# d8ahazard/AudioLab

Hardware: AMD Instinct MI355X
Metric: stems*realtime-factor (44.1kHz stereo) (higher is better)
Workload: dtype bf16; 1 GPU; MDX-Net UVR 4-stem (4x TFC-TDF U-Net L=11 g=48 dim_f=3072 dim_t=256 n_fft=6144), 300 s 44.1 kHz stereo in total, margin chunker, windows/launch=52; stems=4

## Files before the change

audiolab_amd/csrc/tdfnet.hip:

```cpp
#include "mma.h"
#include <alsep_gfx950_asm.h>

#include <map>
#include <type_traits>

namespace {

constexpr int kThreads = 256;

template <typename T> struct Vec16;
template <> struct Vec16<float> { static constexpr int N = 4; };
template <> struct Vec16<bf16_t> { static constexpr int N = 8; };
__device__ __forceinline__ void store_vec(float* p, const float* y) { *reinterpret_cast<float4*>(p) = make_float4(y[0], y[1], y[2], y[3]); }
__device__ __forceinline__ void store_vec(bf16_t* p, const float* y) {
    bf16x8 q;
#pragma unroll
    for (int e = 0; e < 8; ++e) q[e] = (bf16_t)y[e];
    *reinterpret_cast<bf16x8*>(p) = q;
}
__device__ __forceinline__ void load_vec(const float* p, float* x) {
    const float4 q = *reinterpret_cast<const float4*>(p);
    x[0] = q.x; x[1] = q.y; x[2] = q.z; x[3] = q.w;
}
__device__ __forceinline__ void load_vec(const bf16_t* p, float* x) {
// ... 1652 lines not shown
#pragma unroll
            for (int mi = 0; mi < 3; ++mi) acc[u][ni][mi] = f32x4{0.f, 0.f, 0.f, 0.f};

    const int trow = l15 >> 2, tcol = (l15 & 3) * 4;
    const bf16_t* xlane = ring + (4 * lq + trow) * Tc::UC + tcol;
    auto mma_unit = [&](int u, const bf16x8 (&xf)[3], int par, int ks) {
#pragma unroll
        for (int ni = 0; ni < 3; ++ni)
#pragma unroll
            for (int mi = 0; mi < 3; ++mi) mma_step(acc[u][ni][mi], xf[ni], wf[(ALSEP_TDF_ABL & 1) ? 0 : par][ks][mi]);
    };
#define ALSEP_TDFW_STEP(it_, S_, P_)                                                              \
    do {                                                                                          \
        wait_vmcnt<Tc::GLDS>();                 \
        if ((it_) + 1 >= ntile) wait_vmcnt<0>();          \
        barrier_nodrain();                  \
        if ((it_) + 1 < ntile && !(ALSEP_TDF_ABL & 1)) issue_w((it_) + 1, 1 - (P_));              \
        if ((it_) + 2 < ntile && !(ALSEP_TDF_ABL & 4)) issue_x((it_) + 2, ((S_) + 2) % 3);        \
        const bf16_t* xs_ = xlane + (size_t)(S_) * Tc::STAGE_ELEMS;                               \
        bf16x8 xa[3], xb[3];                                                                      \
        tdfw_read_x<0, 0>(xa, xs_);                                                               \
        tdfw_read_x<0, 1>(xb, xs_);                                                               \
        lds_read_tr16_wait_n<6>();  mma_unit(0, xa, P_, 0);                                       \
        tdfw_read_x<0, 2>(xa, xs_);                                                               \
        lds_read_tr16_wait_n<6>();  mma_unit(1, xb, P_, 0);                                       \
        tdfw_read_x<0, 3>(xb, xs_);                                                               \
        lds_read_tr16_wait_n<6>();  mma_unit(2, xa, P_, 0);                                       \
        tdfw_read_x<1, 0>(xa, xs_);                                                               \
        lds_read_tr16_wait_n<6>();  mma_unit(3, xb, P_, 0);                                       \
        tdfw_read_x<1, 1>(xb, xs_);                                                               \
        lds_read_tr16_wait_n<6>();  mma_unit(0, xa, P_, 1);                                       \
        tdfw_read_x<1, 2>(xa, xs_);                                                               \
        lds_read_tr16_wait_n<6>();  mma_unit(1, xb, P_, 1);                                       \
        tdfw_read_x<1, 3>(xb, xs_);                                                               \
        lds_read_tr16_wait_n<6>();  mma_unit(2, xa, P_, 1);                                       \
        lds_read_tr16_wait_n<0>();  mma_unit(3, xb, P_, 1);                                       \
    } while (0)
    issue_x(0, 0);
    issue_w(0, 0);
    if (1 < ntile) issue_x(1, 1);
    for (int it = 0; it < ntile; it += 6) {
        ALSEP_TDFW_STEP(it, 0, 0);
        if (it + 1 < ntile) ALSEP_TDFW_STEP(it + 1, 1, 1);
        if (it + 2 < ntile) ALSEP_TDFW_STEP(it + 2, 2, 0);
        if (it + 3 < ntile) ALSEP_TDFW_STEP(it + 3, 0, 1);
        if (it + 4 < ntile) ALSEP_TDFW_STEP(it + 4, 1, 0);
        if (it + 5 < ntile) ALSEP_TDFW_STEP(it + 5, 2, 1);
    }
#undef ALSEP_TDFW_STEP
    wait_vmcnt<0>();
#pragma unroll
    for (int i = 0; i < 12; ++i) keep_vgprs_live(wf[i / 6][(i / 3) % 2][i % 3]);
    barrier_nodrain();

    float* stg = reinterpret_cast<float*>(alsep_smem) + (size_t)wave * (Tc::TR * Tc::SS);
    bf16_t* frow = reinterpret_cast<bf16_t*>(alsep_smem + Tc::stage_bytes) + (size_t)wave * (Tc::TR * Tc::FS);
    float* fwl = reinterpret_cast<float*>(alsep_smem + Tc::stage_bytes + Tc::final_bytes) + wave * Tc::FWN;
    float fw[3], fbs[4];
    if (FINAL) {
#pragma unroll
        for (int j = 0; j < 3; ++j) fw[j] = FW[j * 64 + lane];
#pragma unroll
        for (int r = 0; r < 4; ++r) fbs[r] = FB[r];
    }
    float bvv[3];
#pragma unroll
    for (int mi = 0; mi < 3; ++mi) bvv[mi] = bias ? bias[rowblk * Tc::TR + mi * 16 + l15] : 0.f;
    auto unit_base = [&](int u) {
        const int64_t U = u0 + u;
        return ((U / upc) * M + rowblk * Tc::TR) * (int64_t)C + (int)(U % upc) * Tc::UC;
    };
    unsigned loff[5];
#pragma unroll
    for (int it = 0; it < 5; ++it) {
        const int gidx = it * 64 + lane;
        loff[it] = (unsigned)(((gidx / 6) * C + (gidx % 6) * 8) * (int)sizeof(bf16_t));
    }
    constexpr int PF = RESIDUAL ? RPF : 0;
    bf16x8 rr[Tc::UN][5];
    auto load_res = [&](int u) {
        const ALSEP_GLOBAL char* rb = opaque_uniform_gptr(reinterpret_cast<const char*>(R + unit_base(u)));
#pragma unroll
        for (int it = 0; it < 5; ++it)
            if (it * 64 + lane < Tc::TR * 6) rr[u][it] = *reinterpret_cast<const ALSEP_GLOBAL bf16x8*>(rb + loff[it]);
    };
    if (RESIDUAL && !(ALSEP_TDF_ABL & 2)) {
#pragma unroll
        for (int u = 0; u < PF && u < Tc::UN; ++u) {
            load_res(u);
            if (FINAL && u == 0) {
#pragma unroll
                for (int j = 0; j < 3; ++j) fwl[j * 64 + lane] = fw[j];
            }
        }
    }
#pragma unroll
    for (int u = 0; u < Tc::UN; ++u) {
        const int cb = (int)((u0 + u) % upc) * Tc::UC;
        if (RESIDUAL && u + PF < Tc::UN && !(ALSEP_TDF_ABL & 2)) load_res(u + PF);
        ALSEP_GLOBAL char* yb = const_cast<ALSEP_GLOBAL char*>(opaque_uniform_gptr(reinterpret_cast<const char*>(Y + unit_base(u))));
#pragma unroll
        for (int ni = 0; ni < 3; ++ni) {
            const f32x4 sc = *reinterpret_cast<const f32x4*>(scale + cb + ni * 16 + 4 * lq);
            const f32x4 sh = *reinterpret_cast<const f32x4*>(shift + cb + ni * 16 + 4 * lq);
#pragma unroll
            for (int mi = 0; mi < 3; ++mi) {
                f32x4 v;
#pragma unroll
                for (int r = 0; r < 4; ++r) v[r] = fmaxf(fmaf(acc[u][ni][mi][r] + bvv[mi], sc[r], sh[r]), 0.f);
                *reinterpret_cast<f32x4*>(stg + (mi * 16 + l15) * Tc::SS + ni * 16 + 4 * lq) = v;
            }
        }
        __builtin_amdgcn_wave_barrier();
#pragma unroll
        for (int it = 0; it < 5; ++it) {
            const int gidx = it * 64 + lane;
            const int fr = gidx / 6, cg = gidx % 6;
            if (gidx < Tc::TR * 6) {
                const f32x4 lo = *reinterpret_cast<const f32x4*>(stg + fr * Tc::SS + cg * 8);
                const f32x4 hi = *reinterpret_cast<const f32x4*>(stg + fr * Tc::SS + cg * 8 + 4);
                float y[8] = {lo[0], lo[1], lo[2], lo[3], hi[0], hi[1], hi[2], hi[3]};
                if (RESIDUAL) {
#pragma unroll
                    for (int e = 0; e < 8; ++e) y[e] += (float)rr[u][it][e];
                }
                bf16x8 q;
#pragma unroll
                for (int e = 0; e < 8; ++e) q[e] = (bf16_t)y[e];
                if (FINAL) *reinterpret_cast<bf16x8*>(frow + fr * Tc::FS + cg * 8) = q;
                else stream_store(reinterpret_cast<ALSEP_GLOBAL bf16x8*>(yb + loff[it]), q);
            }
        }
        __builtin_amdgcn_wave_barrier();
        if (FINAL) {
            const int frl = lane < Tc::TR ? lane : Tc::TR - 1;
            float y[4] = {fbs[0], fbs[1], fbs[2], fbs[3]};
#pragma unroll 2
            for (int ci = 0; ci < Tc::UC; ci += 8) {
                const bf16x8 xv = *reinterpret_cast<const bf16x8*>(frow + frl * Tc::FS + ci);
#pragma unroll
                for (int r = 0; r < 4; ++r) {
                    const f32x4 w0 = *reinterpret_cast<const f32x4*>(fwl + r * Tc::UC + ci);
                    const f32x4 w1 = *reinterpret_cast<const f32x4*>(fwl + r * Tc::UC + ci + 4);
#pragma unroll
                    for (int e = 0; e < 4; ++e) y[r] = fmaf(w0[e], (float)xv[e], y[r]);
#pragma unroll
                    for (int e = 0; e < 4; ++e) y[r] = fmaf(w1[e], (float)xv[4 + e], y[r]);
                }
            }
#pragma unroll
            for (int r = 0; r < 4; ++r) y[r] *= falpha;
            if (lane < Tc::TR) store4(FOUT + (((u0 + u) * M + rowblk * Tc::TR + lane) << 2), y);
            __builtin_amdgcn_wave_barrier();
        }
    }
}

struct Ds48 { static constexpr int C = 48, M = 96, MS = M + 4, K = 192, MT = 6, KS = 6; };
__device__ __forceinline__ vec16 lds_read16_align8(const bf16_t* p) {
    struct alignas(8) half16 { uint32_t w[2]; };
    const half16 a = *reinterpret_cast<const half16*>(p), b = *reinterpret_cast<const half16*>(p + 4);
    vec16 v;
    v.w[0] = a.w[0]; v.w[1] = a.w[1]; v.w[2] = b.w[0]; v.w[3] = b.w[1];
    return v;
}

__global__ void __launch_bounds__(kThreads, 1)
ds48_stream_kernel(const bf16_t* __restrict__ X, bf16_t* __restrict__ Y, const bf16_t* __restrict__ Wf,
                   const float* __restrict__ scale, const float* __restrict__ shift, int64_t npix, int Tp, int Fp) {
    typedef Ds48 D;
    const int tid = threadIdx.x, lane = tid & 63, wave = tid >> 6;
    const int l15 = lane & 15, lq = lane >> 4;
    bf16_t* stg = reinterpret_cast<bf16_t*>(alsep_smem) + (size_t)wave * 64 * D::MS;
    bf16x8 wf[D::MT][D::KS];
#pragma unroll
    for (int mt = 0; mt < D::MT; ++mt)
#pragma unroll
        for (int ks = 0; ks < D::KS; ++ks)
            wf[mt][ks] = *reinterpret_cast<const bf16x8*>(Wf + ((size_t)(mt * D::KS + ks) * 64 + lane) * 8);
    float sc[D::MT][4], sh[D::MT][4];
#pragma unroll
    for (int mt = 0; mt < D::MT; ++mt)
#pragma unroll
        for (int r = 0; r < 4; ++r) { sc[mt][r] = scale[mt * 16 + 4 * lq + r]; sh[mt][r] = shift[mt * 16 + 4 * lq + r]; }
    const int64_t ntile = npix / 64;
    for (int64_t tile = (int64_t)blockIdx.x * 4 + wave; tile < ntile; tile += (int64_t)gridDim.x * 4) {
        const int64_t p0 = tile * 64;
        const int64_t fp0 = p0 % Fp, tp = (p0 / Fp) % Tp, bb = p0 / ((int64_t)Fp * Tp);
        const bf16_t* xrow = X + ((bb * 2 * Tp + 2 * tp) * (2 * (int64_t)Fp) + 2 * fp0) * D::C;
        f32x4 acc[D::MT][4];
#pragma unroll
        for (int mt = 0; mt < D::MT; ++mt)
#pragma unroll
            for (int ni = 0; ni < 4; ++ni) acc[mt][ni] = f32x4{0.f, 0.f, 0.f, 0.f};
#pragma unroll
        for (int ks = 0; ks < D::KS; ++ks) {
            const int k = ks * 32 + lq * 8;
            const int dy = k / (2 * D::C), rem = k % (2 * D::C);
            bf16x8 xf[4];
#pragma unroll
            for (int ni = 0; ni < 4; ++ni)
                xf[ni] = *reinterpret_cast<const bf16x8*>(xrow + (int64_t)dy * (2 * (int64_t)Fp * D::C) + (int64_t)(ni * 16 + l15) * (2 * D::C) + rem);
#pragma unroll
            for (int mt = 0; mt < D::MT; ++mt)
#pragma unroll
                for (int ni = 0; ni < 4; ++ni) mma_step(acc[mt][ni], wf[mt][ks], xf[ni]);
        }
#pragma unroll
        for (int mt = 0; mt < D::MT; ++mt)
#pragma unroll
            for (int ni = 0; ni < 4; ++ni) {
                float y[4];
#pragma unroll
                for (int r = 0; r < 4; ++r) y[r] = fmaxf(fmaf(acc[mt][ni][r], sc[mt][r], sh[mt][r]), 0.f);
                store4(stg + (ni * 16 + l15) * D::MS + mt * 16 + 4 * lq, y);
            }
        __builtin_amdgcn_wave_barrier();
        bf16_t* yrow = Y + p0 * D::M;
#pragma unroll
        for (int it = 0; it < 64 * D::M / 8 / 64; ++it) {
            const int gidx = it * 64 + lane;
            *reinterpret_cast<vec16*>(yrow + (size_t)gidx * 8) = lds_read16_align8(stg + (gidx / (D::M / 8)) * D::MS + (gidx % (D::M / 8)) * 8);
        }
        __builtin_amdgcn_wave_barrier();
    }
}

template <int C_> struct DsSplitCfg {
    static constexpr int C = C_, M = C_ + 48, MS = M + 4, K = 4 * C_, MT = M / 16, KS = K / 32, MTW = (MT + 3) / 4;
    static_assert(M % 16 == 0 && K % 32 == 0, "ds stream geometry");
};
template <int C_, int OCC>
__global__ void __launch_bounds__(kThreads, OCC)
ds_split_stream_kernel(const bf16_t* __restrict__ X, bf16_t* __restrict__ Y, const bf16_t* __restrict__ Wf,
                       const float* __restrict__ scale, const float* __restrict__ shift, int64_t npix, int Tp, int Fp) {
    typedef DsSplitCfg<C_> D;
    const int tid = threadIdx.x, lane = tid & 63, wave = tid >> 6;
    const int l15 = lane & 15, lq = lane >> 4;
    bf16_t* stg = reinterpret_cast<bf16_t*>(alsep_smem);
    bf16x8 wf[D::MTW][D::KS];
#pragma unroll
    for (int j = 0; j < D::MTW; ++j) {
        const int mt = wave + 4 * j;
#pragma unroll
        for (int ks = 0; ks < D::KS; ++ks)
            wf[j][ks] = mt < D::MT ? *reinterpret_cast<const bf16x8*>(Wf + ((size_t)(mt * D::KS + ks) * 64 + lane) * 8) : bf16x8{};
    }
    const int64_t ntile = npix / 64;
    for (int64_t tile = blockIdx.x; tile < ntile; tile += gridDim.x) {
        const int64_t p0 = tile * 64;
        const int64_t fp0 = p0 % Fp, tp = (p0 / Fp) % Tp, bb = p0 / ((int64_t)Fp * Tp);
        const bf16_t* xrow = X + ((bb * 2 * Tp + 2 * tp) * (2 * (int64_t)Fp) + 2 * fp0) * D::C;
        f32x4 acc[D::MTW][4];
#pragma unroll
        for (int j = 0; j < D::MTW; ++j)
#pragma unroll
            for (int ni = 0; ni < 4; ++ni) acc[j][ni] = f32x4{0.f, 0.f, 0.f, 0.f};
#pragma unroll
        for (int ks = 0; ks < D::KS; ++ks) {
            const int k = ks * 32 + lq * 8;
            const int dy = k / (2 * D::C), rem = k % (2 * D::C);
            bf16x8 xf[4];
#pragma unroll
            for (int ni = 0; ni < 4; ++ni)
                xf[ni] = *reinterpret_cast<const bf16x8*>(xrow + (int64_t)dy * (2 * (int64_t)Fp * D::C) + (int64_t)(ni * 16 + l15) * (2 * D::C) + rem);
#pragma unroll
            for (int j = 0; j < D::MTW; ++j)
                if (wave + 4 * j < D::MT) {
#pragma unroll
                    for (int ni = 0; ni < 4; ++ni) mma_step(acc[j][ni], wf[j][ks], xf[ni]);
                }
        }
#pragma unroll
        for (int j = 0; j < D::MTW; ++j) {
            const int mt = wave + 4 * j;
            if (mt < D::MT) {
                const f32x4 scv = *reinterpret_cast<const f32x4*>(scale + mt * 16 + 4 * lq);
                const f32x4 shv = *reinterpret_cast<const f32x4*>(shift + mt * 16 + 4 * lq);
#pragma unroll
                for (int ni = 0; ni < 4; ++ni) {
                    float y[4];
#pragma unroll
                    for (int r = 0; r < 4; ++r) y[r] = fmaxf(fmaf(acc[j][ni][r], scv[r], shv[r]), 0.f);
                    store4(stg + (ni * 16 + l15) * D::MS + mt * 16 + 4 * lq, y);
                }
            }
        }
        __syncthreads();
        bf16_t* yrow = Y + p0 * D::M;
        for (int it = tid; it < 64 * D::M / 8; it += kThreads)
            *reinterpret_cast<vec16*>(yrow + (size_t)it * 8) = lds_read16_align8(stg + (it / (D::M / 8)) * D::MS + (it % (D::M / 8)) * 8);
        __syncthreads();
    }
}

template <int CIN, int C2_, int NI_> struct UsCfg {
    static constexpr int C = CIN, C2 = C2_, NI = NI_, PX = 16 * NI_, MT = C2_ / 16, KS = (CIN + 31) / 32;
    static constexpr int PS = C2_ + 4;
    static constexpr size_t lds_bytes = 2 * (size_t)(2 * PX) * PS * sizeof(float);
    static_assert(C2_ % 16 == 0 && CIN % 8 == 0 && (2 * 2 * PX * (C2_ / 8)) % kThreads == 0, "us stream geometry");
};
template <int CIN, int C2_, int NI_, int OCC = 1>
__global__ void __launch_bounds__(kThreads, OCC)
us_stream_kernel(const bf16_t* __restrict__ X, bf16_t* __restrict__ Y, const bf16_t* __restrict__ Wf,
                 const float* __restrict__ scale, const float* __restrict__ shift, const bf16_t* __restrict__ skip,
                 int64_t npix, int Tp, int Fp) {
// ... 954 lines not shown
template <int KC, int BN>
int run_conv_split_tw(alsep_ctx* ctx, const ConvLayer& L, const float* X, float* Y, int64_t B, int Th, int Fw) {
    if (Fw >= 32) return launch_conv_split<KC, BN, 32>(ctx, L, X, Y, B, Th, Fw);
    return launch_conv_split<KC, BN, 16>(ctx, L, X, Y, B, Th, Fw);
}
int run_conv_split(alsep_ctx* ctx, const ConvLayer& L, const float* X, float* Y, int64_t B, int Th, int Fw) {
    return L.split == 24 ? run_conv_split_tw<24, 48>(ctx, L, X, Y, B, Th, Fw) : run_conv_split_tw<16, 16>(ctx, L, X, Y, B, Th, Fw);
}
int run_conv_split(alsep_ctx* ctx, const ConvLayer&, const bf16_t*, bf16_t*, int64_t, int, int) {
    return alsep_fail(ctx, ALSEP_ERR_STATE, "split contraction is a float32 mode");
}
#endif

template <typename T>
int run_conv(alsep_ctx* ctx, const ConvLayer& L, const T* X, T* Y, int64_t B, int Th, int Fw, const void* zero_page) {
#ifndef ALSEP_F16_TU
    if (L.split) return run_conv_split(ctx, L, X, Y, B, Th, Fw);
#endif
    if (L.dma_path) return run_conv_dma(ctx, L, X, Y, (const T*)zero_page, B, Th, Fw);
    if (conv_uses_main<T>(L.cin, L.cout)) return run_conv_tw<T, ConvSel<T>::KC, ConvSel<T>::BN>(ctx, L, X, Y, B, Th, Fw);
    return run_conv_tw<T, ConvSel16<T>::KC, ConvSel16<T>::BN>(ctx, L, X, Y, B, Th, Fw);
}

int pix_stream_enabled() {
    static const int v = [] { const char* e = getenv("ALSEP_PIX_STREAM"); return e ? atoi(e) : 1; }();
    return v;
}
int run_pix_stream(alsep_ctx* ctx, int mode, const GemmLayer& L, const bf16_t* X, bf16_t* Y, const bf16_t* skip, int64_t ncols,
                   int Tp, int Fp) {
    ProfScope prof(ctx, ALSEP_PROF_PIX);
    const int64_t ntile = ncols / 64;
    if (mode == PIX_DS && L.M == Ds48::M) {
        const size_t lds = 4 * 64 * Ds48::MS * sizeof(bf16_t);
        const int64_t gx = std::min<int64_t>(ceil_div64(ntile, 4), 256);
        hipLaunchKernelGGL(ds48_stream_kernel, dim3((unsigned)gx), dim3(kThreads), lds, ctx->stream, X, Y, (const bf16_t*)L.wfrag.p,
                           (const float*)L.scale.p, (const float*)L.shift.p, ncols, Tp, Fp);
        note_launch(ctx, "ds48_stream_kernel");
    } else if (mode == PIX_DS && L.M == DsSplitCfg<96>::M) {
        const size_t lds = 64 * DsSplitCfg<96>::MS * sizeof(bf16_t);
        const int64_t gx = std::min<int64_t>(ntile, 512);
        hipLaunchKernelGGL((ds_split_stream_kernel<96, 2>), dim3((unsigned)gx), dim3(kThreads), lds, ctx->stream, X, Y,
                           (const bf16_t*)L.wfrag.p, (const float*)L.scale.p, (const float*)L.shift.p, ncols, Tp, Fp);
        note_launch(ctx, "ds_split_stream_kernel<96>");
    } else if (mode == PIX_DS) {
        const size_t lds = 64 * DsSplitCfg<144>::MS * sizeof(bf16_t);
        const int64_t gx = std::min<int64_t>(ntile, 512);
        hipLaunchKernelGGL((ds_split_stream_kernel<144, 1>), dim3((unsigned)gx), dim3(kThreads), lds, ctx->stream, X, Y,
                           (const bf16_t*)L.wfrag.p, (const float*)L.scale.p, (const float*)L.shift.p, ncols, Tp, Fp);
        note_launch(ctx, "ds_split_stream_kernel<144>");
    } else {
#define ALSEP_US(CIN_, C2_, NI_, OCC_, GX_)                                                                                 \
    {                                                                                                                       \
        typedef UsCfg<CIN_, C2_, NI_> U;                                                                                    \
        ALSEP_HIP(ctx, hipFuncSetAttribute((const void*)us_stream_kernel<CIN_, C2_, NI_, OCC_>,                             \
                                           hipFuncAttributeMaxDynamicSharedMemorySize, (int)U::lds_bytes));                 \
        const int64_t gx = std::min<int64_t>(ncols / U::PX, GX_);                                                           \
        hipLaunchKernelGGL((us_stream_kernel<CIN_, C2_, NI_, OCC_>), dim3((unsigned)gx), dim3(kThreads), U::lds_bytes,      \
                           ctx->stream, X, Y, (const bf16_t*)L.wfrag.p, (const float*)L.scale.p, (const float*)L.shift.p,   \
                           skip, ncols, Tp, Fp);                                                                            \
        note_launch(ctx, "us_stream_kernel<" #CIN_ "," #C2_ ">");                                                          \
    }
        if (L.K == 96) ALSEP_US(96, 48, 4, 1, 512)
        else if (L.K == 144) ALSEP_US(144, 96, 2, 2, 512)
        else ALSEP_US(192, 144, 2, 1, 256)
#undef ALSEP_US
    }
    note_launch(ctx, mode == PIX_DS ? "ds_stream_kernel" : "us_stream_kernel");
    ALSEP_LAUNCH_CHECK(ctx, "pix stream kernel");
    return ALSEP_OK;
}
int run_pix_stream(alsep_ctx* ctx, int, const GemmLayer&, const float*, float*, const float*, int64_t, int, int) {
    return alsep_fail(ctx, ALSEP_ERR_STATE, "streaming ds/us path is bf16 only");
}

#ifndef ALSEP_F16_TU
template <int MODE>
int run_pix_split(alsep_ctx* ctx, const GemmLayer& L, const float* X, float* Y, const float* skip, int64_t ncols, int Tp, int Fp, int C, int C2) {
    typedef GemmSCfg Gc;
    const int64_t gx = ceil_div64(ncols, Gc::BC);
    if (gx > 0x7fffffff) return alsep_fail(ctx, ALSEP_ERR_ARG, "pix_gemm: too many column tiles");
    ALSEP_HIP(ctx, hipFuncSetAttribute((const void*)pix_gemm_f32s_kernel<MODE>, hipFuncAttributeMaxDynamicSharedMemorySize, (int)Gc::lds_bytes));
    ProfScope prof(ctx, ALSEP_PROF_PIX);
    const int nrb = L.Mp / Gc::BR;
    const int fast = (nrb > 1 && gx % 8 == 0 && gx * nrb <= 0x7fffffff) ? nrb : 0;
    hipLaunchKernelGGL((pix_gemm_f32s_kernel<MODE>), fast ? dim3((unsigned)(gx * nrb)) : dim3((unsigned)gx, nrb), dim3(kThreads), Gc::lds_bytes,
                       ctx->stream, X, Y, (const hs_t*)L.w.p, (const float*)L.scale.p, (const float*)L.shift.p, skip, L.M, L.Mp, L.K, L.Kp, ncols,
                       Tp, Fp, C, C2, L.range_flag, fast);
    ALSEP_LAUNCH_CHECK(ctx, "pix_gemm_f32s_kernel");
    return ALSEP_OK;
}
template <int MODE>
int run_pix_split(alsep_ctx* ctx, const GemmLayer&, const bf16_t*, bf16_t*, const bf16_t*, int64_t, int, int, int, int) {
    return alsep_fail(ctx, ALSEP_ERR_STATE, "split contraction is a float32 mode");
}
int run_tdf_split(alsep_ctx* ctx, const GemmLayer& L, const float* X, float* Y, const float* R, int64_t BT, int C) {
    typedef GemmSCfg Gc;
    const int64_t nunits = BT * (C / 16);
    const int64_t gx = ceil_div64(nunits, 8);
    if (gx > 0x7fffffff) return alsep_fail(ctx, ALSEP_ERR_ARG, "tdf_gemm: too many column tiles");
    const float* bias = L.has_bias ? (const float*)L.bias.p : nullptr;
    ProfScope prof(ctx, ALSEP_PROF_TDF);
    const int nrb = L.Mp / Gc::BR;
    const int fast = (nrb > 1 && gx % 8 == 0 && gx * nrb <= 0x7fffffff) ? nrb : 0;
    const dim3 grid = fast ? dim3((unsigned)(gx * nrb)) : dim3((unsigned)gx, nrb);
    if (R) {
        ALSEP_HIP(ctx, hipFuncSetAttribute((const void*)tdf_gemm_f32s_kernel<true>, hipFuncAttributeMaxDynamicSharedMemorySize, (int)Gc::lds_bytes));
        hipLaunchKernelGGL((tdf_gemm_f32s_kernel<true>), grid, dim3(kThreads), Gc::lds_bytes, ctx->stream, X, Y, (const hs_t*)L.w.p, bias,
                           (const float*)L.scale.p, (const float*)L.shift.p, R, L.M, L.Mp, L.K, L.Kp, nunits, C, L.range_flag, fast);
    } else {
        ALSEP_HIP(ctx, hipFuncSetAttribute((const void*)tdf_gemm_f32s_kernel<false>, hipFuncAttributeMaxDynamicSharedMemorySize, (int)Gc::lds_bytes));
        hipLaunchKernelGGL((tdf_gemm_f32s_kernel<false>), grid, dim3(kThreads), Gc::lds_bytes, ctx->stream, X, Y, (const hs_t*)L.w.p, bias,
                           (const float*)L.scale.p, (const float*)L.shift.p, R, L.M, L.Mp, L.K, L.Kp, nunits, C, L.range_flag, fast);
    }
    ALSEP_LAUNCH_CHECK(ctx, "tdf_gemm_f32s_kernel");
    return ALSEP_OK;
}
int run_tdf_split(alsep_ctx* ctx, const GemmLayer&, const bf16_t*, bf16_t*, const bf16_t*, int64_t, int) {
    return alsep_fail(ctx, ALSEP_ERR_STATE, "split contraction is a float32 mode");
}
#endif

template <typename T, int MODE>
int run_pix(alsep_ctx* ctx, const GemmLayer& L, const T* X, T* Y, const T* skip, int64_t ncols, int Tp, int Fp, int C, int C2) {
    typedef GemmCfg<T> Gc;
#ifndef ALSEP_F16_TU
    if (L.split) return run_pix_split<MODE>(ctx, L, X, Y, skip, ncols, Tp, Fp, C, C2);
#endif
    if (L.wfrag.p && pix_stream_enabled() && Fp % 64 == 0) return run_pix_stream(ctx, MODE, L, X, Y, skip, ncols, Tp, Fp);
    const int64_t gx = ceil_div64(ncols, Gc::BC);
    if (gx > 0x7fffffff) return alsep_fail(ctx, ALSEP_ERR_ARG, "pix_gemm: too many column tiles");
    ProfScope prof(ctx, ALSEP_PROF_PIX);
    hipLaunchKernelGGL((pix_gemm_kernel<T, MODE>), dim3((unsigned)gx, L.Mp / Gc::BR), dim3(kThreads), Gc::lds_bytes,
                       ctx->stream, X, Y, (const T*)L.w.p, (const float*)L.scale.p, (const float*)L.shift.p, skip,
                       L.M, L.K, L.Kp, ncols, Tp, Fp, C, C2);
    ALSEP_LAUNCH_CHECK(ctx, "pix_gemm_kernel");
    return ALSEP_OK;
}

int tdf_wide_mode() {
    static const int v = [] { const char* e = getenv("ALSEP_TDF_WIDE"); return e ? atoi(e) : 1; }();
    return v;
}
struct FinalFold {
    const float* w;
    const float* b;
    void* out;
    float alpha;
    bool done;
};
int tdf_final_mode() {
    static const int v = [] { const char* e = getenv("ALSEP_TDF_FINAL"); return e ? atoi(e) : 1; }();
    return v;
}
template <int WM>
int launch_tdf_wide(alsep_ctx* ctx, const GemmLayer& L, const bf16_t* X, bf16_t* Y, const bf16_t* R, int64_t nunits, int C,
                    FinalFold* fin) {
    typedef TdfWide<WM> Tc;
    const int64_t gx = ceil_div64(nunits, Tc::UN);
    if (gx > 0x7fffffff) return alsep_fail(ctx, ALSEP_ERR_ARG, "tdf: too many column tiles");
    const float* bias = L.has_bias ? (const float*)L.bias.p : nullptr;
    static const int yfast = [] { const char* e = getenv("ALSEP_TDF_YFAST"); return e ? atoi(e) : 1; }();
    const int nrb = L.M / Tc::BM;
    const int nyb = (yfast && nrb > 1 && gx % 8 == 0 && gx * nrb <= 0x7fffffff) ? nrb : 0;
    const dim3 grid = nyb ? dim3((unsigned)(gx * nrb)) : dim3((unsigned)gx, nrb);
    ProfScope prof(ctx, ALSEP_PROF_TDF);
    static const int rpf = [] { const char* e = getenv("ALSEP_TDF_RPF"); return e ? atoi(e) : 2; }();
    if (WM == 4 && R && rpf != 0 && fin && C == Tc::UC && tdf_final_mode()) {
        ALSEP_HIP(ctx, hipFuncSetAttribute((const void*)tdf_bf16_wide_kernel<4, true, 2, true>,
                                           hipFuncAttributeMaxDynamicSharedMemorySize, (int)TdfWide<4>::lds_bytes));
        hipLaunchKernelGGL((tdf_bf16_wide_kernel<4, true, 2, true>), grid, dim3(TdfWide<4>::THREADS), TdfWide<4>::lds_bytes,
                           ctx->stream, X, Y, (const bf16_t*)L.wwide.p, bias, (const float*)L.scale.p, (const float*)L.shift.p, R,
                           L.M, L.K, nunits, C, nyb, fin->w, fin->b, (bf16_t*)fin->out, fin->alpha);
        fin->done = true;
        note_launch(ctx, "tdf_bf16_wide_kernel<res,final>");
    } else if (R && rpf == 0) {
        ALSEP_HIP(ctx, hipFuncSetAttribute((const void*)tdf_bf16_wide_kernel<WM, true, 0>,
                                           hipFuncAttributeMaxDynamicSharedMemorySize, (int)Tc::lds_bytes));
        hipLaunchKernelGGL((tdf_bf16_wide_kernel<WM, true, 0>), grid, dim3(Tc::THREADS), Tc::lds_bytes, ctx->stream, X, Y,
                           (const bf16_t*)L.wwide.p, bias, (const float*)L.scale.p, (const float*)L.shift.p, R, L.M, L.K,
                           nunits, C, nyb, (const float*)nullptr, (const float*)nullptr, (bf16_t*)nullptr, 0.f);
    } else if (R) {
        ALSEP_HIP(ctx, hipFuncSetAttribute((const void*)tdf_bf16_wide_kernel<WM, true>,
                                           hipFuncAttributeMaxDynamicSharedMemorySize, (int)Tc::lds_bytes));
        hipLaunchKernelGGL((tdf_bf16_wide_kernel<WM, true>), grid, dim3(Tc::THREADS), Tc::lds_bytes, ctx->stream, X, Y,
                           (const bf16_t*)L.wwide.p, bias, (const float*)L.scale.p, (const float*)L.shift.p, R, L.M, L.K,
                           nunits, C, nyb, (const float*)nullptr, (const float*)nullptr, (bf16_t*)nullptr, 0.f);
    } else {
        ALSEP_HIP(ctx, hipFuncSetAttribute((const void*)tdf_bf16_wide_kernel<WM, false>,
                                           hipFuncAttributeMaxDynamicSharedMemorySize, (int)Tc::lds_bytes));
        hipLaunchKernelGGL((tdf_bf16_wide_kernel<WM, false>), grid, dim3(Tc::THREADS), Tc::lds_bytes, ctx->stream, X, Y,
                           (const bf16_t*)L.wwide.p, bias, (const float*)L.scale.p, (const float*)L.shift.p, R, L.M, L.K,
                           nunits, C, nyb, (const float*)nullptr, (const float*)nullptr, (bf16_t*)nullptr, 0.f);
    }
    note_launch(ctx, R ? "tdf_bf16_wide_kernel<res>" : "tdf_bf16_wide_kernel<nores>");
    ALSEP_LAUNCH_CHECK(ctx, "tdf_bf16_wide_kernel");
    return ALSEP_OK;
}

int run_tdf_dma(alsep_ctx* ctx, const GemmLayer& L, const bf16_t* X, bf16_t* Y, const bf16_t* R, const bf16_t* zp,
                int64_t BT, int C, FinalFold* fin) {
    typedef TdfB16 Tc;
    const int64_t nunits = BT * (C / Tc::UC);
    if (L.wwide.p && tdf_wide_mode() && L.K % 64 == 0 && nunits % 4 == 0) {
        const int mode = tdf_wide_mode();
        const bool can8 = L.M % 384 == 0;
        const bool use8 = mode == 8 ? can8 : (mode == 4 ? false : (can8 && L.M == 384 && !R));
        return use8 ? launch_tdf_wide<8>(ctx, L, X, Y, R, nunits, C, nullptr) : launch_tdf_wide<4>(ctx, L, X, Y, R, nunits, C, fin);
    }
    const int64_t gx = ceil_div64(nunits, Tc::UN);
    if (gx > 0x7fffffff) return alsep_fail(ctx, ALSEP_ERR_ARG, "tdf: too many column tiles");
    const float* bias = L.has_bias ? (const float*)L.bias.p : nullptr;
    ProfScope prof(ctx, ALSEP_PROF_TDF);
    const dim3 grid((unsigned)gx, L.Mp / Tc::BM);
    if (R)
        hipLaunchKernelGGL((tdf_bf16_kernel<true>), grid, dim3(kThreads), Tc::lds_bytes, ctx->stream, X, Y, (const bf16_t*)L.w.p,
                           bias, (const float*)L.scale.p, (const float*)L.shift.p, R, zp, L.M, L.K, L.Kp, nunits, C);
    else
        hipLaunchKernelGGL((tdf_bf16_kernel<false>), grid, dim3(kThreads), Tc::lds_bytes, ctx->stream, X, Y, (const bf16_t*)L.w.p,
                           bias, (const float*)L.scale.p, (const float*)L.shift.p, R, zp, L.M, L.K, L.Kp, nunits, C);
    ALSEP_LAUNCH_CHECK(ctx, "tdf_bf16_kernel");
    return ALSEP_OK;
}
int run_tdf_dma(alsep_ctx* ctx, const GemmLayer&, const float*, float*, const float*, const float*, int64_t, int, FinalFold*) {
    return alsep_fail(ctx, ALSEP_ERR_STATE, "LDS-DMA TDF path is bf16 only");
}

template <typename T>
int run_tdf(alsep_ctx* ctx, const GemmLayer& L, const T* X, T* Y, const T* R, int64_t BT, int C, const void* zero_page,
            FinalFold* fin = nullptr) {
    typedef GemmCfg<T> Gc;
#ifndef ALSEP_F16_TU
    if (L.split) return run_tdf_split(ctx, L, X, Y, R, BT, C);
#endif
    if (L.dma_path) return run_tdf_dma(ctx, L, X, Y, R, (const T*)zero_page, BT, C, fin);
    const int64_t nunits = BT * (C / 16);
    const int64_t gx = ceil_div64(nunits, 8);
    if (gx > 0x7fffffff) return alsep_fail(ctx, ALSEP_ERR_ARG, "tdf_gemm: too many column tiles");
    const float* bias = L.has_bias ? (const float*)L.bias.p : nullptr;
    ProfScope prof(ctx, ALSEP_PROF_TDF);
    if (R)
        hipLaunchKernelGGL((tdf_gemm_kernel<T, true>), dim3((unsigned)gx, L.Mp / Gc::BR), dim3(kThreads), Gc::lds_bytes,
                           ctx->stream, X, Y, (const T*)L.w.p, bias, (const float*)L.scale.p, (const float*)L.shift.p, R,
                           L.M, L.K, L.Kp, nunits, C);
    else
        hipLaunchKernelGGL((tdf_gemm_kernel<T, false>), dim3((unsigned)gx, L.Mp / Gc::BR), dim3(kThreads), Gc::lds_bytes,
                           ctx->stream, X, Y, (const T*)L.w.p, bias, (const float*)L.scale.p, (const float*)L.shift.p, R,
                           L.M, L.K, L.Kp, nunits, C);
    ALSEP_LAUNCH_CHECK(ctx, "tdf_gemm_kernel");
    return ALSEP_OK;
}

template <typename T>
int run_block(alsep_ctx* ctx, const alsep_net* net, const Block& blk, const T* cur, T* a, T* b, T* h, T* dest,
              int64_t B, int Th, int Fw, int c, FinalFold* fin = nullptr) {
    const T* src = cur;
    T* pp[2] = {a, b};
    int rc;
    const int l = (int)blk.tfc.size();
    for (int j = 0; j < l; ++j) {
        T* dst = pp[j & 1];
        if ((rc = run_conv<T>(ctx, blk.tfc[j], src, dst, B, Th, Fw, net->zero_page.p))) return rc;
        src = dst;
    }
    if (blk.tdf.size() == 2) {
        if ((rc = run_tdf<T>(ctx, blk.tdf[0], src, h, (const T*)nullptr, B * Th, c, net->zero_page.p))) return rc;
        return run_tdf<T>(ctx, blk.tdf[1], h, dest, src, B * Th, c, net->zero_page.p, fin);
    }
    return run_tdf<T>(ctx, blk.tdf[0], src, dest, src, B * Th, c, net->zero_page.p, fin);
}

size_t align256(size_t v) { return (v + 255) & ~(size_t)255; }

struct WsLayout {
    size_t p0, p1, p2, h, total;
    std::vector<size_t> skip;
};

WsLayout ws_layout(const alsep_net* net, int64_t B) {
    const alsep_net_config& cfg = net->cfg;
    const size_t es = cfg.dtype == ALSEP_F32 ? 4 : 2;
    WsLayout w;
    const size_t s0 = align256((size_t)B * cfg.dim_t * cfg.dim_f * cfg.g * es);
    size_t off = 0;
    w.p0 = off; off += s0;
    w.p1 = off; off += s0;
    w.p2 = off; off += s0;
    w.h = off;  off += align256(cfg.bn > 0 ? s0 / cfg.bn : 16);
    int c = cfg.g;
    size_t t = cfg.dim_t, f = cfg.dim_f;
    for (int i = 0; i < net->n; ++i) {
        w.skip.push_back(off);
        off += align256((size_t)B * t * f * c * es);
        c += cfg.g; t /= 2; f /= 2;
    }
    w.total = off;
    return w;
}

struct PcmFront {
    const alsep_plan* plan;
    const float* pcm;
    int64_t ch_stride, chunk_stride;
    int zero_low;
};

template <typename T>
int forward_impl(alsep_ctx* ctx, const alsep_net* net, const T* in, T* out, int64_t B, char* ws, float in_scale,
                 float out_alpha, float out_beta, const PcmFront* front = nullptr) {
    const alsep_net_config& cfg = net->cfg;
    const WsLayout L = ws_layout(net, B);
    T* P[3] = {(T*)(ws + L.p0), (T*)(ws + L.p1), (T*)(ws + L.p2)};
    T* H = (T*)(ws + L.h);
    int Th = cfg.dim_t, Fw = cfg.dim_f, c = cfg.g;
    const int64_t npix0 = B * Th * Fw;
    int rc;
    if (front) {
        if ((rc = ALSEP_TU_NAME(alsep_stft_first_conv)(ctx, front->plan, front->pcm, front->ch_stride, front->chunk_stride, B, P[0],
                                                       (const float*)net->first_w.p, (const float*)net->first_scale.p,
                                                       (const float*)net->first_shift.p, cfg.g, in_scale, front->zero_low)))
            return rc;
// ... 169 lines not shown
```

Baseline: 5906 stems*x_realtime.

## Add persistent TDF residual GEMM kernel that keeps activation tile resident across row blocks

```diff
diff --git a/audiolab_amd/csrc/tdfnet.hip b/audiolab_amd/csrc/tdfnet.hip
--- a/audiolab_amd/csrc/tdfnet.hip
+++ b/audiolab_amd/csrc/tdfnet.hip
@@ -1828,6 +1828,232 @@
             for (int r = 0; r < 4; ++r) y[r] *= falpha;
             if (lane < Tc::TR) store4(FOUT + (((u0 + u) * M + rowblk * Tc::TR + lane) << 2), y);
             __builtin_amdgcn_wave_barrier();
+        }
+    }
+}
+
+struct TdfPersist {
+    static constexpr int WV = 8, TR = 48, BM = TR * WV, UN = 2, UC = 48, BK = 64;
+    static constexpr int THREADS = 64 * WV;
+    static constexpr int STAGE_ELEMS = UN * BK * UC;
+    static constexpr int SS = TdfWide<4>::SS, FS = TdfWide<4>::FS, FWN = TdfWide<4>::FWN;
+    static constexpr size_t stage_bytes = (size_t)WV * TR * SS * sizeof(float);
+    static constexpr size_t bn_bytes = (size_t)UN * 2 * UC * sizeof(float);
+    static constexpr size_t tile_bytes(int nt) { return (size_t)nt * STAGE_ELEMS * sizeof(bf16_t); }
+    static constexpr size_t lds_bytes(int nt, bool fin) { return tile_bytes(nt) + stage_bytes + bn_bytes + (fin ? WV * FWN * sizeof(float) : 0); }
+    static_assert((size_t)TR * FS * sizeof(bf16_t) <= (size_t)TR * SS * sizeof(float), "FINAL: the rounded rows fit in the staging rows");
+};
+
+__device__ __forceinline__ void glds16_base(const ALSEP_GLOBAL char* gbase, unsigned lane_off, void* lds_wave_base) {
+    __builtin_amdgcn_global_load_lds((const ALSEP_GLOBAL void*)(gbase + lane_off), (__attribute__((address_space(3))) void*)lds_wave_base, 16, 0, 0);
+}
+
+template <int NT, bool FINAL>
+__global__ void __launch_bounds__(TdfPersist::THREADS, 1)
+tdf_bf16_persist_kernel(const bf16_t* __restrict__ X, bf16_t* __restrict__ Y, const bf16_t* __restrict__ Wf,
+                        const float* __restrict__ bias, const float* __restrict__ scale, const float* __restrict__ shift,
+                        const bf16_t* __restrict__ R, int M, int64_t nitems, int C,
+                        const float* __restrict__ FW, const float* __restrict__ FB, bf16_t* __restrict__ FOUT, float falpha) {
+    typedef TdfPersist Tc;
+    static_assert(NT % 3 == 0 && NT >= 3, "three weight buffers: a K tile's buffer is the same in every row block");
+    static_assert(Tc::lds_bytes(NT, FINAL) <= 160 * 1024, "LDS of a CU");
+    constexpr int K = NT * Tc::BK;
+    bf16_t* tile = reinterpret_cast<bf16_t*>(alsep_smem);
+    const int tid = threadIdx.x, lane = tid & 63;
+    const int wave = __builtin_amdgcn_readfirstlane(tid >> 6);
+    const int l15 = lane & 15, lq = lane >> 4;
+    float* stg = reinterpret_cast<float*>(alsep_smem + Tc::tile_bytes(NT)) + (size_t)wave * (Tc::TR * Tc::SS);
+    bf16_t* frow = reinterpret_cast<bf16_t*>(stg);
+    float* bnl = reinterpret_cast<float*>(alsep_smem + Tc::tile_bytes(NT) + Tc::stage_bytes);
+    float* fwl = bnl + Tc::UN * 2 * Tc::UC + wave * Tc::FWN;
+    const int ush = C / Tc::UC - 1;
+    const int nrb = M / Tc::BM;
+
+    if (tid < Tc::UN * 2 * Tc::UC) {
+        const int u = tid / (2 * Tc::UC), which = (tid / Tc::UC) & 1, c = tid % Tc::UC;
+        bnl[tid] = (which ? shift : scale)[(u & ush) * Tc::UC + c];
+    }
+    float fbs[4];
+    if (FINAL) {
+#pragma unroll
+        for (int j = 0; j < 3; ++j) fwl[j * 64 + lane] = FW[j * 64 + lane];
+#pragma unroll
+        for (int r = 0; r < 4; ++r) fbs[r] = FB[r];
+    }
+    unsigned loff[5], xoff[3];
+#pragma unroll
+    for (int j = 0; j < 3; ++j) {
+        const int within = j * 64 + lane;
+        xoff[j] = (unsigned)(((within / 6) * C + (within % 6) * 8) * (int)sizeof(bf16_t));
+    }
+#pragma unroll
+    for (int it = 0; it < 5; ++it) {
+        const int gidx = it * 64 + lane;
+        loff[it] = (unsigned)(((gidx / 6) * C + (gidx % 6) * 8) * (int)sizeof(bf16_t));
+    }
+    const unsigned woff = (unsigned)lane * 16u;
+    const int trow = l15 >> 2, tcol = (l15 & 3) * 4;
+    const bf16_t* xlane = tile + (4 * lq + trow) * Tc::UC + tcol;
+
+    bf16x8 wf[3][2][3];
+    auto load_w = [&](int buf, int rowblk, int it) {
+        const ALSEP_GLOBAL char* wp = opaque_uniform_gptr(reinterpret_cast<const char*>(Wf) + ((size_t)rowblk * NT + it) * (6 * 1024));
+#pragma unroll
+        for (int i = 0; i < 6; ++i) wf[buf][i / 3][i % 3] = *reinterpret_cast<const ALSEP_GLOBAL bf16x8*>(wp + woff + i * 1024);
+    };
+
+    for (int64_t item = blockIdx.x; item < nitems; item += gridDim.x) {
+        const int64_t u0 = item * Tc::UN;
+        load_w(0, wave, 0);
+        load_w(1, wave, 1);
+        barrier_nodrain();
+        constexpr int NP = NT * Tc::UN * 6;
+#pragma unroll 1
+        for (int p = wave; p < NP; p += Tc::WV) {
+            {
+                const int tu = p / 6, j = p % 6, it = tu / Tc::UN, u = tu % Tc::UN;
+                const ALSEP_GLOBAL char* src = opaque_uniform_gptr(reinterpret_cast<const char*>(
+                    X + (((u0 + u) >> ush) * K + it * Tc::BK + (j / 3) * 32) * (int64_t)C + (u & ush) * Tc::UC));
+                const int j3 = j % 3;
+                glds16_base(src, j3 == 0 ? xoff[0] : (j3 == 1 ? xoff[1] : xoff[2]), tile + (size_t)p * 64 * 8);
+            }
+        }
+        wait_vmcnt<0>();
+        barrier_nodrain();
+
+        for (int rb = 0; rb < nrb; ++rb) {
+            const int rowblk = rb * Tc::WV + wave;
+            const int rownext = (rb + 1 < nrb ? rb + 1 : rb) * Tc::WV + wave;
+            auto unit_base = [&](int u) {
+                return (((u0 + u) >> ush) * M + rowblk * Tc::TR) * (int64_t)C + (u & ush) * Tc::UC;
+            };
+            f32x4 acc[Tc::UN][3][3];
+#pragma unroll
+            for (int u = 0; u < Tc::UN; ++u)
+#pragma unroll
+                for (int ni = 0; ni < 3; ++ni)
+#pragma unroll
+                    for (int mi = 0; mi < 3; ++mi) acc[u][ni][mi] = f32x4{0.f, 0.f, 0.f, 0.f};
+            bf16x8 rr[Tc::UN][5];
+            float bvv[3];
+            bf16x8 xa[3], xb[3];
+            auto mma_unit = [&](int u, const bf16x8 (&xf)[3], int buf, int ks) {
+#pragma unroll
+                for (int ni = 0; ni < 3; ++ni)
+#pragma unroll
+                    for (int mi = 0; mi < 3; ++mi) mma_step(acc[u][ni][mi], xf[ni], wf[buf][ks][mi]);
+            };
+#pragma unroll
+            for (int it = 0; it < NT; ++it) {
+                if (it + 2 < NT) load_w((it + 2) % 3, rowblk, it + 2);
+                else load_w((it + 2) % 3, rownext, it + 2 - NT);
+                if (it == 0) {
+                    const int ln = FINAL ? opaque_vgpr(lane) : lane;
+                    const unsigned roff4 = FINAL ? (unsigned)((((256 + ln) / 6) * C + ((256 + ln) % 6) * 8) * (int)sizeof(bf16_t)) : loff[4];
+                    const unsigned boff = (unsigned)((ln & 15) * (int)sizeof(float));
+#pragma unroll
+                    for (int u = 0; u < Tc::UN; ++u) {
+                        const ALSEP_GLOBAL char* rp = opaque_uniform_gptr(reinterpret_cast<const char*>(R + unit_base(u)));
+#pragma unroll
+                        for (int g = 0; g < 4; ++g) rr[u][g] = *reinterpret_cast<const ALSEP_GLOBAL bf16x8*>(rp + loff[g]);
+                        if (lane < Tc::TR * 6 - 256) rr[u][4] = *reinterpret_cast<const ALSEP_GLOBAL bf16x8*>(rp + roff4);
+                    }
+#pragma unroll
+                    for (int mi = 0; mi < 3; ++mi) bvv[mi] = 0.f;
+                    if (bias) {
+                        const ALSEP_GLOBAL char* bp = opaque_uniform_gptr(reinterpret_cast<const char*>(bias + rowblk * Tc::TR));
+#pragma unroll
+                        for (int mi = 0; mi < 3; ++mi)
+                            bvv[mi] = *reinterpret_cast<const ALSEP_GLOBAL float*>(bp + boff + mi * 16 * (int)sizeof(float));
+                    }
+                }
+                const bf16_t* xs = xlane + (size_t)it * Tc::STAGE_ELEMS;
+                if (it == 0) {
+                    tdfw_read_x<0, 0>(xa, xs);
+                    tdfw_read_x<0, 1>(xb, xs);
+                }
+                lds_read_tr16_wait_n<6>();  mma_unit(0, xa, it % 3, 0);
+                tdfw_read_x<1, 0>(xa, xs);
+                lds_read_tr16_wait_n<6>();  mma_unit(1, xb, it % 3, 0);
+                tdfw_read_x<1, 1>(xb, xs);
+                if (it + 1 < NT) {
+                    lds_read_tr16_wait_n<6>();  mma_unit(0, xa, it % 3, 1);
+                    tdfw_read_x<0, 0>(xa, xs + Tc::STAGE_ELEMS);
+                    lds_read_tr16_wait_n<6>();  mma_unit(1, xb, it % 3, 1);
+                    tdfw_read_x<0, 1>(xb, xs + Tc::STAGE_ELEMS);
+                } else {
+                    lds_read_tr16_wait_n<6>();  mma_unit(0, xa, it % 3, 1);
+                    lds_read_tr16_wait_n<0>();  mma_unit(1, xb, it % 3, 1);
+                }
+            }
+
+#pragma unroll
+            for (int u = 0; u < Tc::UN; ++u) {
+                ALSEP_GLOBAL char* yb = const_cast<ALSEP_GLOBAL char*>(opaque_uniform_gptr(reinterpret_cast<const char*>(Y + unit_base(u))));
+#pragma unroll
+                for (int ni = 0; ni < 3; ++ni) {
+                    const f32x4 sc = *reinterpret_cast<const f32x4*>(bnl + u * 2 * Tc::UC + ni * 16 + 4 * lq);
+                    const f32x4 sh = *reinterpret_cast<const f32x4*>(bnl + u * 2 * Tc::UC + Tc::UC + ni * 16 + 4 * lq);
+#pragma unroll
+                    for (int mi = 0; mi < 3; ++mi) {
+                        f32x4 v;
+#pragma unroll
+                        for (int r = 0; r < 4; ++r) v[r] = fmaxf(fmaf(acc[u][ni][mi][r] + bvv[mi], sc[r], sh[r]), 0.f);
+                        *reinterpret_cast<f32x4*>(stg + (mi * 16 + l15) * Tc::SS + ni * 16 + 4 * lq) = v;
+                    }
+                }
+                __builtin_amdgcn_wave_barrier();
+                bf16x8 q[5];
+#pragma unroll
+                for (int g = 0; g < 5; ++g) {
+                    const int gidx = g * 64 + lane;
+                    const int fr = gidx / 6, cg = gidx % 6;
+                    if (gidx < Tc::TR * 6) {
+                        const f32x4 lo = *reinterpret_cast<const f32x4*>(stg + fr * Tc::SS + cg * 8);
+                        const f32x4 hi = *reinterpret_cast<const f32x4*>(stg + fr * Tc::SS + cg * 8 + 4);
+                        float y[8] = {lo[0], lo[1], lo[2], lo[3], hi[0], hi[1], hi[2], hi[3]};
+#pragma unroll
+                        for (int e = 0; e < 8; ++e) y[e] += (float)rr[u][g][e];
+#pragma unroll
+                        for (int e = 0; e < 8; ++e) q[g][e] = (bf16_t)y[e];
+                        if (!FINAL) stream_store(reinterpret_cast<ALSEP_GLOBAL bf16x8*>(yb + loff[g]), q[g]);
+                    }
+                }
+                __builtin_amdgcn_wave_barrier();
+                if (FINAL) {
+#pragma unroll
+                    for (int g = 0; g < 5; ++g) {
+                        const int gidx = g * 64 + lane;
+                        if (gidx < Tc::TR * 6) *reinterpret_cast<bf16x8*>(frow + (gidx / 6) * Tc::FS + (gidx % 6) * 8) = q[g];
+                    }
+                    __builtin_amdgcn_wave_barrier();
+                    const int ln = opaque_vgpr(lane);
+                    const int frl = ln < Tc::TR ? ln : Tc::TR - 1;
+                    float y[4] = {fbs[0], fbs[1], fbs[2], fbs[3]};
+#pragma unroll 2
+                    for (int ci = 0; ci < Tc::UC; ci += 8) {
+                        const bf16x8 xv = *reinterpret_cast<const bf16x8*>(frow + frl * Tc::FS + ci);
+#pragma unroll
+                        for (int r = 0; r < 4; ++r) {
+                            const f32x4 w0 = *reinterpret_cast<const f32x4*>(fwl + r * Tc::UC + ci);
+                            const f32x4 w1 = *reinterpret_cast<const f32x4*>(fwl + r * Tc::UC + ci + 4);
+#pragma unroll
+                            for (int e = 0; e < 4; ++e) y[r] = fmaf(w0[e], (float)xv[e], y[r]);
+#pragma unroll
+                            for (int e = 0; e < 4; ++e) y[r] = fmaf(w1[e], (float)xv[4 + e], y[r]);
+                        }
+                    }
+#pragma unroll
+                    for (int r = 0; r < 4; ++r) y[r] *= falpha;
+                    ALSEP_GLOBAL char* fo = const_cast<ALSEP_GLOBAL char*>(
+                        opaque_uniform_gptr(reinterpret_cast<const char*>(FOUT + (((u0 + u) * M + rowblk * Tc::TR) << 2))));
+                    bf16x4 yq;
+#pragma unroll
+                    for (int r = 0; r < 4; ++r) yq[r] = (bf16_t)y[r];
+                    if (ln < Tc::TR) *reinterpret_cast<ALSEP_GLOBAL bf16x4*>(fo + (unsigned)ln * (4u * (unsigned)sizeof(bf16_t))) = yq;
+                    __builtin_amdgcn_wave_barrier();
+                }
+            }
         }
     }
 }
@@ -3088,6 +3314,45 @@
     static const int v = [] { const char* e = getenv("ALSEP_TDF_FINAL"); return e ? atoi(e) : 1; }();
     return v;
 }
+enum { kTdfPersistK384 = 1, kTdfPersistK192 = 2, kTdfPersistFinal = 4 };
+constexpr int kTdfPersistRouted = kTdfPersistK384 | kTdfPersistK192 | kTdfPersistFinal;
+int tdf_persist_mode() {
+    static const int v = [] { const char* e = getenv("ALSEP_TDF_PERSIST"); return e ? atoi(e) : 1; }();
+    return v;
+}
+template <int NT, bool FINAL>
+void launch_tdf_persist_inst(alsep_ctx* ctx, hipError_t& attr, unsigned grid, const GemmLayer& L, const bf16_t* X, bf16_t* Y,
+                             const bf16_t* R, int64_t nitems, int C, const FinalFold* fin) {
+    constexpr int lds = (int)TdfPersist::lds_bytes(NT, FINAL);
+    attr = hipFuncSetAttribute((const void*)tdf_bf16_persist_kernel<NT, FINAL>, hipFuncAttributeMaxDynamicSharedMemorySize, lds);
+    if (attr != hipSuccess) return;
+    hipLaunchKernelGGL((tdf_bf16_persist_kernel<NT, FINAL>), dim3(grid), dim3(TdfPersist::THREADS), lds, ctx->stream, X, Y,
+                       (const bf16_t*)L.wwide.p, L.has_bias ? (const float*)L.bias.p : nullptr, (const float*)L.scale.p,
+                       (const float*)L.shift.p, R, L.M, nitems, C, fin ? fin->w : nullptr, fin ? fin->b : nullptr,
+                       fin ? (bf16_t*)fin->out : nullptr, fin ? fin->alpha : 0.f);
+}
+int launch_tdf_persist(alsep_ctx* ctx, const GemmLayer& L, const bf16_t* X, bf16_t* Y, const bf16_t* R, int64_t nunits, int C,
+                       FinalFold* fin) {
+    static const int cap = [] { const char* e = getenv("ALSEP_TDF_PERSIST_GRID"); return e ? atoi(e) : 0; }();
+    const int64_t nitems = nunits / TdfPersist::UN;
+    int64_t grid = device_cu_count(ctx);
+    if (cap > 0 && cap < grid) grid = cap;
+    if (nitems < grid) grid = nitems;
+    hipError_t attr = hipSuccess;
+    if (fin && L.K == 384) launch_tdf_persist_inst<6, true>(ctx, attr, (unsigned)grid, L, X, Y, R, nitems, C, fin);
+    else if (fin) launch_tdf_persist_inst<3, true>(ctx, attr, (unsigned)grid, L, X, Y, R, nitems, C, fin);
+    else if (L.K == 384) launch_tdf_persist_inst<6, false>(ctx, attr, (unsigned)grid, L, X, Y, R, nitems, C, nullptr);
+    else launch_tdf_persist_inst<3, false>(ctx, attr, (unsigned)grid, L, X, Y, R, nitems, C, nullptr);
+    ALSEP_HIP(ctx, attr);
+    if (fin) {
+        fin->done = true;
+        note_launch(ctx, "tdf_bf16_wide_kernel<res,final>");
+    }
+    note_launch(ctx, "tdf_bf16_wide_kernel<res>");
+    ALSEP_LAUNCH_CHECK(ctx, "tdf_bf16_persist_kernel");
+    return ALSEP_OK;
+}
+
 template <int WM>
 int launch_tdf_wide(alsep_ctx* ctx, const GemmLayer& L, const bf16_t* X, bf16_t* Y, const bf16_t* R, int64_t nunits, int C,
                     FinalFold* fin) {
@@ -3101,7 +3366,15 @@
     const dim3 grid = nyb ? dim3((unsigned)(gx * nrb)) : dim3((unsigned)gx, nrb);
     ProfScope prof(ctx, ALSEP_PROF_TDF);
     static const int rpf = [] { const char* e = getenv("ALSEP_TDF_RPF"); return e ? atoi(e) : 2; }();
-    if (WM == 4 && R && rpf != 0 && fin && C == Tc::UC && tdf_final_mode()) {
+    const bool fold = WM == 4 && R && rpf != 0 && fin && C == Tc::UC && tdf_final_mode();
+    if (WM == 4 && R && rpf != 0 && tdf_wide_mode() == 1 && L.M % TdfPersist::BM == 0 && (C == Tc::UC || C == 2 * Tc::UC) &&
+        (L.K == 384 || L.K == 192)) {
+        const int kind = fold ? kTdfPersistFinal : (L.K == 384 ? kTdfPersistK384 : kTdfPersistK192);
+        const int mode = tdf_persist_mode();
+        if (mode >= 2 || (mode == 1 && (kTdfPersistRouted & kind)))
+            return launch_tdf_persist(ctx, L, X, Y, R, nunits, C, fold ? fin : nullptr);
+    }
+    if (fold) {
         ALSEP_HIP(ctx, hipFuncSetAttribute((const void*)tdf_bf16_wide_kernel<4, true, 2, true>,
                                            hipFuncAttributeMaxDynamicSharedMemorySize, (int)TdfWide<4>::lds_bytes));
         hipLaunchKernelGGL((tdf_bf16_wide_kernel<4, true, 2, true>), grid, dim3(TdfWide<4>::THREADS), TdfWide<4>::lds_bytes,
```

New measurement: 5996 stems*x_realtime (median of 6 runs). 1.02x the previous value.
